# MartinPippel/DAmar

Hardware: AMD Instinct MI355X
Metric: aligned base-pairs/sec (daligner block-vs-block) (higher is better)
Workload: dtype int32

## Files before the change

damar_amd/csrc/kernels/kernels.h:

```cpp
#ifndef DAMAR_KERNELS_H
#define DAMAR_KERNELS_H

#include "dev_common.h"

size_t damar_scan_workspace_bytes(u64 n);
void   damar_exclusive_scan_u32(const u32 *in, u32 *out, u64 n, void *work, u64 *total_dev, hipStream_t st);
#define DAMAR_SCAN_TILE 4096
void   damar_tile_offsets_u32(const u32 *in, u64 n, void *work, u64 *total_dev, hipStream_t st);
void   damar_scan_tile_counts(u32 *tcount, u32 ntiles, u64 *total_dev, hipStream_t st);
size_t damar_sort_workspace_bytes(u64 n);
void   damar_sort_set_threads(int threads);
const u32 *damar_sort_error_word(const void *work);
int    damar_radix_sort_keys_u64(u64 *k0, u64 *k1, u64 n, int lobit, int hibit, void *work, hipStream_t st);
void   damar_radix_sort_split_u64(u64 *k0, u64 *k1, u64 n, int lobit, int hibit, u32 *ohi, u32 *olo, void *work,
                                  hipStream_t st);
int    damar_radix_sort_u32(u32 *k0, u32 *v0, u32 *k1, u32 *v1, u64 n, int nbits, void *work, hipStream_t st);
int    damar_radix_sort_keys_u32(u32 *k0, u32 *k1, u64 n, int nbits, void *work, hipStream_t st);
int    damar_radix_sort_u64(u64 *k0, u32 *v0, u64 *k1, u32 *v1, u64 n, int nbits, void *work, hipStream_t st);

typedef struct
{ const u8  *bases;
  const u32 *pk;
  u32        rbias;
  const u32 *boff;
// ... 64 lines not shown
  int  self, comp, identity;
  u32  limit;
  DevBlock ablk, bblk;
  int  pbits, abits;
  int  dbits;
} MergeArgs;

typedef struct { u32 b0, b1, ja, ia;
                 u32 sh, pad[3]; } MergeTile;

size_t damar_merge_workspace_bytes(u32 alen);
u32   *damar_merge_tile_counts(void *work, u32 alen);
u32    damar_merge_tiles(u32 alen);
void   damar_launch_merge_count(const MergeArgs *m, void *work, unsigned long long *gram, u32 ngram, hipStream_t st);
void damar_launch_merge_emit(const MergeArgs *m, void *work, u64 nhits, u64 *keys, u32 *vals, u32 *pid, hipStream_t st);
void damar_launch_pair_heads_ids(const u32 *pids, u64 nhits, int abits, int minhit, int nshift,
                                 u64 *send, u64 *bits, void *scan_work, u64 *total_dev, u32 *heads, hipStream_t st);
void damar_launch_pair_bitmap(const u32 *pids, const u32 *heads, u32 nheads, int abits, u32 b_lo, u32 b_hi, u32 *bitmap,
                              hipStream_t st);
void damar_launch_seed_cut_count(const u64 *keys, u64 nhits, int pbits, const u32 *bitmap, u32 *tcount, u64 *total_dev,
                                 hipStream_t st);
void damar_launch_seed_cut_scatter(const u64 *keys, const u32 *vals, u64 nhits, int pbits, const u32 *bitmap,
                                   const u32 *toff, u64 *okeys, u32 *ovals, hipStream_t st);
void damar_launch_pair_heads(const u64 *keys, u64 nhits, int pbits, int abits, int minhit, int nshift,
                             u64 *send , u64 *bits, void *scan_work, u64 *total_dev,
                             u32 *heads, hipStream_t st);
void damar_launch_pair_work(u64 *keys, const u32 *vals, u64 nhits, int ppos, int dbits, int abits, int minhit, int nshift,
                            u64 *send , u64 *bits, void *scan_work, u64 *total_dev ,
                            int binshift, int kmer, int hitmin, u32 b_lo, u32 b_hi, int unsorted, hipStream_t st);
void damar_launch_order_runs(u64 *keys, u64 nhits, int ppos, int dbits, const u32 *work, u32 nwork, hipStream_t st);
// ... 146 lines not shown
```

damar_amd/csrc/kernels/radix_sort.hip:

```cpp
#include <atomic>
#include <type_traits>
#include "dev_common.h"
#include "kernels.h"

SEED_PRIO_VAR(g_sort_prio, 1)
SEED_PRIO_SETTER(damar_sort_set_prio, g_sort_prio)

#ifndef OS_THREADS
#define OS_THREADS 1024
#endif
#ifndef OS_MINW
#define OS_MINW    4
#endif
#ifndef OS_RANK_LDS
#define OS_RANK_LDS 1
#endif
#define OS_MINTILE (256 * 8)
#define OS_MAXPASS 8

#define OH_ITEMS   16

#define LB_COUNT   1u
#define LB_PREFIX  2u
#define LB_SPINS   (1u << 24)
#ifndef LB_AHEAD
#define LB_AHEAD   8
#endif

#define WS_HIST    256
#define WS_CTR     (256 + OS_MAXPASS * 256 * 4)
#define WS_LB      16384

template <typename GT> __device__ __forceinline__ GT lb_load(const GT *p)
{ return __hip_atomic_load(p, __ATOMIC_RELAXED, __HIP_MEMORY_SCOPE_AGENT); }
template <typename GT> __device__ __forceinline__ void lb_store(GT *p, GT v)
{ __hip_atomic_store(p, v, __ATOMIC_RELAXED, __HIP_MEMORY_SCOPE_AGENT); }

__device__ __forceinline__ u32 os_scan256(u32 v, u32 *lds4)
{ const int l = lane_id(), w = threadIdx.x >> 6;
  const u32 inc = (u32) wave_incl_scan_i((int) v);
  if (l == 63 && w < 4) lds4[w] = inc;
  __syncthreads();
  u32 base = 0;
  for (int i = 0; i < 4; i++)
    if (i < w) base += lds4[i];
  __syncthreads();
  return base + inc - v;
}


#define OH_THREADS 1024
// ... 439 lines not shown
```

damar_amd/csrc/kernels/seed_merge.hip:

```cpp
#include "dev_common.h"
#include "kernels.h"

SEED_PRIO_VAR(g_merge_prio, 0)
SEED_PRIO_SETTER(damar_merge_set_prio, g_merge_prio)


__device__ __forceinline__ u32 count_below(const u32 *__restrict__ bpos, u32 jb, u32 ib, u32 bound)
{ u32 a = jb, b = ib;
  while (a < b)
    { u32 m = (a + b) >> 1;
      if (bpos[m] < bound) a = m + 1; else b = m;
    }
  return a - jb;
}


#ifndef MT_PER
#define MT_PER  4
#endif
#define MT_A    (MT_PER * 256)
#define MT_BCAP (3 * MT_A)
#define MT_HITS 4
#define MT_NBK  2048

template <typename CodeT>
__device__ __forceinline__ u32 lower_bound_c(const CodeT *c, u32 lo, u32 hi, CodeT x)
{ while (lo < hi)
    { const u32 mid = (lo + hi) >> 1;
      if (c[mid] < x) lo = mid + 1; else hi = mid;
    }
  return lo;
}
template <typename CodeT>
__device__ __forceinline__ u32 upper_bound_c(const CodeT *c, u32 lo, u32 hi, CodeT x)
{ while (lo < hi)
    { const u32 mid = (lo + hi) >> 1;
      if (c[mid] <= x) lo = mid + 1; else hi = mid;
    }
  return lo;
}

#define MT_SMP 8192
template <typename CodeT>
__global__ __launch_bounds__(256)
void merge_tiles(MergeArgs m, u32 ntiles, MergeTile *__restrict__ tiles)
{ SEED_PRIO(g_merge_prio);
  constexpr u32 NS = sizeof(CodeT) == 4 ? MT_SMP : MT_SMP / 2;
  __shared__ CodeT smp[NS];
  const CodeT *acode = (const CodeT *) m.acode, *bcode = (const CodeT *) m.bcode;
  const u32 stride = (m.blen + NS - 1) / NS;
  if (m.blen > 0)
    for (u32 j = threadIdx.x; j < NS; j += 256)
      { const u64 e = (u64) (j + 1) * stride - 1;
        smp[j] = bcode[e < m.blen ? (u32) e : m.blen - 1];
      }
  __syncthreads();
  const u32 t = blockIdx.x * 256u + threadIdx.x;
  if (t >= ntiles)
    return;
  const u32 a0 = t * (u32) MT_A, a1 = min(m.alen, a0 + (u32) MT_A);
  const CodeT c0 = acode[a0], c1 = acode[a1 - 1];
// ... 73 lines not shown
  return count_below(m.bpos, jb, jb + nb, bound);
}

__device__ __forceinline__ u64 block_sum_u64(u64 v, u64 *red)
{ for (int o = 32; o > 0; o >>= 1)
    { const u32 lo = (u32) __shfl_xor((int) (u32) v, o), hi = (u32) __shfl_xor((int) (u32) (v >> 32), o);
      v += ((u64) hi << 32) | lo;
    }
  __syncthreads();
  if (lane_id() == 0) red[threadIdx.x >> 6] = v;
  __syncthreads();
  return red[0] + red[1] + red[2] + red[3];
}

template <typename CodeT, bool INLDS>
__device__ __forceinline__ void merge_sweep_tile(const MergeArgs &m, const MergeTile tl, const u32 tile,
                                                 u32 *__restrict__ tcount, u32 *__restrict__ cnt, u32 *__restrict__ jbg,
                                                 unsigned long long *__restrict__ gram, u32 ngram,
                                                 CodeT *sb, u32 *loc, u32 *sjb, u32 *sw4, u64 *red)
{ const CodeT *acode = (const CodeT *) m.acode, *bcode = (const CodeT *) m.bcode;
  const int l = lane_id(), w = threadIdx.x >> 6;
  const u32 a0 = tile * (u32) MT_A, a1 = min(m.alen, a0 + (u32) MT_A), nat = a1 - a0;
  const u32 nbt = tl.b1 - tl.b0;
  const u32 e0 = threadIdx.x * MT_PER;
  const int nv = (e0 >= nat) ? 0 : (int) min((u32) MT_PER, nat - e0);

  constexpr u32 VPK = 16 / sizeof(CodeT);
  typedef CodeT VecT __attribute__((ext_vector_type(16 / sizeof(CodeT))));
  CodeT a[MT_PER];
  if (nv == MT_PER)
    {
// ... 242 lines not shown
#pragma unroll
      for (int k = 0; k < 4; k++)
        { vc[k] = n[k];  vj[k] = tl.b0 + jb[k]; }
      *(V4 *) (cnt + a0 + e0) = vc;
      *(V4 *) (jbg + a0 + e0) = vj;
    }
  else
    {
#pragma unroll
      for (int k = 0; k < MT_PER; k++)
        if (k < nv)
          { cnt[a0 + e0 + k] = n[k];
            jbg[a0 + e0 + k] = tl.b0 + jb[k];
          }
    }
}

static_assert(MT_BCAP + 16 < (1 << 16), "a packed entry holds the piece-relative start and the hits in 16 bits each");
struct MergeFastArgs
{ const void *acode, *bcode;
  const u32  *apos, *bpos;
  u32 alen, blen;
  int self, identity, comp, rpbits;
};

template <typename CodeT>
__global__ __launch_bounds__(256, 8)
void merge_fast(MergeFastArgs m, MergeTile *__restrict__ tiles, u32 *__restrict__ tcount, u32 *__restrict__ cnt)
{ SEED_PRIO(g_merge_prio);
  __shared__ __attribute__((aligned(16))) CodeT sb[MT_BCAP + 16 / sizeof(CodeT)];
  __shared__ __attribute__((aligned(16))) u16 first[MT_NBK];
  __shared__ u32 wsum[4];
  __shared__ u32 deep;
  const CodeT *acode = (const CodeT *) m.acode, *bcode = (const CodeT *) m.bcode;
  const u32 tile = blockIdx.x;
  const MergeTile tl = tiles[tile];
  const u32 a0 = tile * (u32) MT_A, a1 = min(m.alen, a0 + (u32) MT_A), nat = a1 - a0;
  const u32 nbt = tl.b1 - tl.b0;
  if (nbt > MT_BCAP || (m.self && m.rpbits == 0))
    { if (threadIdx.x == 0)
        tiles[tile].pad[0] = 1;
      return;
    }
  const u32 e0 = threadIdx.x * MT_PER;
  const int nv = (e0 >= nat) ? 0 : (int) min((u32) MT_PER, nat - e0);
  const u32 sh = tl.sh, nmax = tl.pad[1];
  constexpr u32 VPK = 16 / sizeof(CodeT);
  typedef CodeT VecT __attribute__((ext_vector_type(16 / sizeof(CodeT))));
  typedef u32 V4 __attribute__((ext_vector_type(4)));

  const CodeT c0 = acode[a0];
  CodeT a[MT_PER];
  if (nv == MT_PER)
    {
#pragma unroll
      for (int q = 0; q < MT_PER / (int) VPK; q++)
        { const VecT v = ((const VecT *) (acode + a0 + e0))[q];
#pragma unroll
// ... 34 lines not shown
    for (int r = 0; r < MT_BCAP / (int) VPK / 256 + 1; r++)
      { const u32 x = threadIdx.x + (u32) r * 256;
        if (x < nvec)
          ((VecT *) sb)[x] = v[r];
      }
  }
  const CodeT *B = sb + shf;
  __syncthreads();
  for (u32 j = threadIdx.x; j < nbt; j += 256)
    { const u32 bk = (u32) ((B[j] - c0) >> sh);
      if (j == 0 || (u32) ((B[j - 1] - c0) >> sh) != bk)
        first[bk] = (u16) j;
    }
  __syncthreads();

  u32 jb[MT_PER], n[MT_PER];
  u32 longest = 0;
#pragma unroll
  for (int k = 0; k < MT_PER; k++)
    { jb[k] = 0;  n[k] = 0;
      if (k < nv)
        { const CodeT c = a[k];
          if (k > 0 && c == a[k - 1])
            { jb[k] = jb[k - 1];  n[k] = n[k - 1]; }
          else
            { u32 p = first[(u32) ((c - c0) >> sh)];
              if (p != 0xffffu)
                { int steps = 0;
                  while (p < nbt && B[p] < c)
                    { p += 1;
                      if (++steps == 4) { p = lower_bound_c<CodeT>(B, p, nbt, c);  break; }
// ... 20 lines not shown
        if (n[k] > 0)
          { const u32 p = m.apos[a0 + e0 + k], ra = p >> rp;
            u32 bound = m.identity ? (m.comp ? (ra + 1) << rp : p) : ra << rp;
            if (!(m.identity && m.comp && ((ra + 1) >> (32 - rp)) != 0))
              n[k] = count_below(m.bpos, tl.b0 + jb[k], tl.b0 + jb[k] + n[k], bound);
          }
    }
#pragma unroll
  for (int k = 0; k < MT_PER; k++)
    sum += n[k];
  sum = (u32) wave_sum_i((int) sum);
  if (lane_id() == 0)
    wsum[threadIdx.x >> 6] = sum;
  __syncthreads();
  if (deep)
    { if (threadIdx.x == 0)
        tiles[tile].pad[0] = 1;
      return;
    }
  if (threadIdx.x == 0)
    { tcount[tile] = wsum[0] + wsum[1] + wsum[2] + wsum[3];
      tiles[tile].pad[2] = 1;
    }
  if (nv == MT_PER && MT_PER == 4)
    { V4 vc;
#pragma unroll
      for (int k = 0; k < 4; k++)
        vc[k] = (n[k] << 16) | jb[k];
      *(V4 *) (cnt + a0 + e0) = vc;
    }
  else
    {
#pragma unroll
      for (int k = 0; k < MT_PER; k++)
        if (k < nv)
          cnt[a0 + e0 + k] = (n[k] << 16) | jb[k];
    }
}

template <typename CodeT>
__global__ __launch_bounds__(256, 8)
void merge_sweep(MergeArgs m, const MergeTile *__restrict__ tiles, u32 *__restrict__ tcount, u32 *__restrict__ cnt,
                 u32 *__restrict__ jbg, unsigned long long *__restrict__ gram, u32 ngram, int only_flagged)
{ SEED_PRIO(g_merge_prio);
  __shared__ __attribute__((aligned(16))) CodeT sb[MT_BCAP + 16 / sizeof(CodeT)];
  __shared__ u32 loc[MT_A + 1];
  __shared__ u32 sjb[2];
  __shared__ u32 sw4[4];
  __shared__ u64 red[4];
  const MergeTile tl = tiles[blockIdx.x];
  if (only_flagged && tl.pad[0] == 0)
    return;
  if (tl.b1 - tl.b0 <= MT_BCAP)
    merge_sweep_tile<CodeT, true>(m, tl, blockIdx.x, tcount, cnt, jbg, gram, ngram, sb, loc, sjb, sw4, red);
  else
    merge_sweep_tile<CodeT, false>(m, tl, blockIdx.x, tcount, cnt, jbg, gram, ngram, sb, loc, sjb, sw4, red);
}

__global__ __launch_bounds__(256, 8)
void merge_emit(MergeArgs m, const MergeTile *__restrict__ tiles, const u32 *__restrict__ cnt, const u32 *__restrict__ jbg,
                const u32 *__restrict__ toff, u64 nhits, u64 *__restrict__ keys, u32 *__restrict__ vals, u32 *__restrict__ pid)
{ SEED_PRIO(g_merge_prio);
  __shared__ u32 loc[MT_A + 1];
  __shared__ u32 sjb[MT_A];
  __shared__ u32 sw4[4];
  const int l = lane_id(), w = threadIdx.x >> 6;
  const u32 tile = blockIdx.x;
  const u32 a0 = tile * (u32) MT_A, a1 = min(m.alen, a0 + (u32) MT_A), nat = a1 - a0;
  const u32 e0 = threadIdx.x * MT_PER;
  const u64 h0 = toff[tile];
  const u64 hn = (tile + 1 < gridDim.x) ? (u64) toff[tile + 1] : nhits;
  if (hn == h0)
    return;
  u32 n[MT_PER], s = 0;
  const bool packed = tiles[tile].pad[2] != 0;
  const u32 pb0 = tiles[tile].b0;
#pragma unroll
  for (int k = 0; k < MT_PER; k++)
    { const bool ok = e0 + k < nat;
      const u32 w = ok ? cnt[a0 + e0 + k] : 0;
      n[k] = packed ? w >> 16 : w;
      sjb[e0 + k] = !ok ? 0 : packed ? pb0 + (w & 0xffffu) : jbg[a0 + e0 + k];
      s += n[k];
    }
  u32 inc = (u32) wave_incl_scan_i((int) s);
  if (l == 63) sw4[w] = inc;
  __syncthreads();
  u32 ex = inc - s;
  for (int i = 0; i < 4; i++)
    if (i < w) ex += sw4[i];
#pragma unroll
  for (int k = 0; k < MT_PER; k++)
    { loc[e0 + k] = ex;
      ex += n[k];
    }
  if (threadIdx.x == 255)
    loc[MT_A] = ex;
  __syncthreads();
  const u32 T = loc[MT_A];
  for (u32 t0 = threadIdx.x; t0 < T; t0 += 256 * MT_HITS)
    { u32 ai[MT_HITS], bi[MT_HITS], pa[MT_HITS], pb[MT_HITS];
#pragma unroll
      for (int x = 0; x < MT_HITS; x++)
        { const u32 t = t0 + (u32) x * 256;
          u32 lo = 0, hi = MT_A;
          if (t < T)
            while (hi - lo > 1)
              { const u32 mid = (lo + hi) >> 1;
                if (loc[mid] <= t) lo = mid; else hi = mid;
              }
          ai[x] = a0 + lo;
          bi[x] = (t < T) ? sjb[lo] + (t - loc[lo]) : 0;
        }
#pragma unroll
      for (int x = 0; x < MT_HITS; x++)
        { const bool ok = t0 + (u32) x * 256 < T;
          pa[x] = ok ? m.apos[ai[x]] : 0;
          pb[x] = ok ? m.bpos[bi[x]] : 0;
        }
      u32 ra[MT_HITS], rb[MT_HITS], xa[MT_HITS], xb[MT_HITS];
      if (m.ablk.rpbits && m.bblk.rpbits)
        {
#pragma unroll
          for (int x = 0; x < MT_HITS; x++)
            { ra[x] = pa[x] >> m.ablk.rpbits;  xa[x] = pa[x] & ((1u << m.ablk.rpbits) - 1u);
              rb[x] = pb[x] >> m.bblk.rpbits;  xb[x] = pb[x] & ((1u << m.bblk.rpbits) - 1u);
            }
        }
      else
        {
#pragma unroll
          for (int x = 0; x < MT_HITS; x++)
            { pos_decode(m.ablk, pa[x], &ra[x], &xa[x]);
              pos_decode(m.bblk, pb[x], &rb[x], &xb[x]);
            }
        }
// ... 4 lines not shown
          if (t < T && h < nhits)
            { const u64 key = ((u64) rb[x] << (m.abits + m.pbits)) | ((u64) ra[x] << m.pbits) | (u64) xa[x];
              if (m.dbits)
                keys[h] = (key << m.dbits) | (u64) xb[x];
              else
                { keys[h] = key;
                  vals[h] = (u32) ((int) xa[x] - (int) xb[x]);
                }
              if (pid != NULL)
                pid[h] = (rb[x] << m.abits) | ra[x];
            }
        }
    }
}

static size_t mw_tiles(u32 alen)  { return ((size_t) alen + MT_A - 1) / MT_A; }
static size_t mw_off_counts(u32 alen) { return (mw_tiles(alen) * sizeof(MergeTile) + 255) & ~(size_t) 255; }
static size_t mw_off_cnt(u32 alen)    { return mw_off_counts(alen) + (((mw_tiles(alen) + 1) * sizeof(u32) + 255) & ~(size_t) 255); }
static size_t mw_off_jb(u32 alen)     { return mw_off_cnt(alen) + (((size_t) alen * sizeof(u32) + 255) & ~(size_t) 255); }

size_t damar_merge_workspace_bytes(u32 alen)
{ return mw_off_jb(alen) + (((size_t) alen * sizeof(u32) + 255) & ~(size_t) 255); }

u32 *damar_merge_tile_counts(void *work, u32 alen) { return (u32 *) ((char *) work + mw_off_counts(alen)); }

u32 damar_merge_tiles(u32 alen) { return (u32) mw_tiles(alen); }

void damar_launch_merge_count(const MergeArgs *m, void *work, unsigned long long *gram, u32 ngram, hipStream_t st)
{ if (m->alen == 0)
    return;
  const u32 ntiles = (u32) mw_tiles(m->alen);
  MergeTile *tiles = (MergeTile *) work;
  u32 *tcount = damar_merge_tile_counts(work, m->alen);
  u32 *cnt = (u32 *) ((char *) work + mw_off_cnt(m->alen)), *jb = (u32 *) ((char *) work + mw_off_jb(m->alen));
  static int general = -1;
  if (general < 0)
    general = getenv("DAMAR_MERGE_GENERAL") != NULL;
  const bool fast = gram == NULL && !general;
  MergeFastArgs f;
  f.acode = m->acode;  f.bcode = m->bcode;  f.apos = m->apos;  f.bpos = m->bpos;  f.alen = m->alen;  f.blen = m->blen;
  f.self = m->self;  f.identity = m->identity;  f.comp = m->comp;  f.rpbits = m->ablk.rpbits;
  if (m->wide)
    { hipLaunchKernelGGL(merge_tiles<u64>, dim3((ntiles + 255) / 256), dim3(256), 0, st, *m, ntiles, tiles);
      if (fast)
        hipLaunchKernelGGL(merge_fast<u64>, dim3(ntiles), dim3(256), 0, st, f, tiles, tcount, cnt);
      hipLaunchKernelGGL(merge_sweep<u64>, dim3(ntiles), dim3(256), 0, st, *m, tiles, tcount, cnt, jb, gram, ngram, fast ? 1 : 0);
    }
  else
    { hipLaunchKernelGGL(merge_tiles<u32>, dim3((ntiles + 255) / 256), dim3(256), 0, st, *m, ntiles, tiles);
      if (fast)
        hipLaunchKernelGGL(merge_fast<u32>, dim3(ntiles), dim3(256), 0, st, f, tiles, tcount, cnt);
      hipLaunchKernelGGL(merge_sweep<u32>, dim3(ntiles), dim3(256), 0, st, *m, tiles, tcount, cnt, jb, gram, ngram, fast ? 1 : 0);
    }
}

void damar_launch_merge_emit(const MergeArgs *m, void *work, u64 nhits, u64 *keys, u32 *vals, u32 *pid, hipStream_t st)
{ if (nhits == 0)
    return;
  const u32 ntiles = (u32) mw_tiles(m->alen);
  const u32 *toff = damar_merge_tile_counts(work, m->alen);
  const u32 *cnt = (const u32 *) ((char *) work + mw_off_cnt(m->alen)), *jb = (const u32 *) ((char *) work + mw_off_jb(m->alen));
  hipLaunchKernelGGL(merge_emit, dim3(ntiles), dim3(256), 0, st, *m, (const MergeTile *) work, cnt, jb, toff, nhits, keys, vals, pid);
}

#define SCREEN_MAX   48
#define SCREEN_PANEL 50000
template <typename K>
__global__ __launch_bounds__(64)
void slice_ends(const K *__restrict__ keys, u64 nhits, int bshift, int nshift, u64 *__restrict__ send)
{ const int nthr = 1 << nshift, t = threadIdx.x;
  if (t >= nthr)
    return;
  u64 e;
  if (t == nthr - 1)
    e = nhits;
  else
    { e = (nhits * (u64) (t + 1)) >> nshift;
      if (e > 0)
// ... 763 lines not shown
```

damar_amd/csrc/shim.hip:

```cpp
#include <algorithm>
#include <vector>
#include <deque>
#include <string>
#include <thread>
#include <atomic>
#include <mutex>
#include <condition_variable>
#include <functional>
#include <string.h>
#include <unistd.h>

#include "kernels/dev_common.h"
#include <ctype.h>
#include "kernels/kernels.h"

extern "C" {
#include "damar_filter.h"
#include "damar_hip.h"
#include "host/damar_host.h"
}

#define MAXGRAM 10000

static void die(void)
// ... 1730 lines not shown
  m.abits = std::max(1, ilog2_ceil((u64) ablock->nreads));
  int bbits = std::max(1, ilog2_ceil((u64) bblock->nreads));
  if (m.pbits + m.abits + bbits > 64)
    { fprintf(stderr, "damar: FATAL: seed key needs %d bits (> 64)\n", m.pbits + m.abits + bbits);
      die();
    }
  { static int pack_on = -1;
    if (pack_on < 0)
      { const char *e = getenv("DAMAR_PACK_SEEDS");
        pack_on = e ? atoi(e) : 1;
      }
    const int db = std::max(1, ilog2_ceil((u64) bblock->maxlen + 1));
    m.dbits = (pack_on && m.pbits + m.abits + bbits + db <= 64) ? db : 0;
  }

  const u32 mtiles = damar_merge_tiles(alen);
  void *mw;
  u32  *tcount;
  u64  *tot;
  u64   total = 0;

  if (Q_flush > 0)
    { Q_ms[3] += now_ms() - Q_flush;  Q_flush = 0; }
  Q_seg[3] += now_ms() - f->t_entry;
  tick(0);
  arena_reserve(&G_work, pad256(damar_merge_workspace_bytes(alen)) + pad256(damar_scan_workspace_bytes(mtiles)) + 4096);
  mw = arena_take(&G_work, damar_merge_workspace_bytes(alen));
  tcount = damar_merge_tile_counts(mw, alen);
  tot = (u64 *) arena_take(&G_work, 64);
  void *mscw = arena_take(&G_work, damar_scan_workspace_bytes(mtiles));
  damar_launch_merge_count(&m, mw, NULL, 0, G_st);
  stage("merge_count");
  damar_exclusive_scan_u32(tcount, tcount, mtiles, mscw, tot, G_st);
  stage("merge_scan");
  HIP_CHECK(hipMemcpyAsync(&total, tot, sizeof(u64), hipMemcpyDeviceToHost, G_st));
  stream_wait(G_st);
  if (MEM_LIMIT > 0)
    {
      int   limit = MAXGRAM;
      int64 avail = (int64) (MEM_LIMIT - (uint64) (sizeof_db(ablock) + sizeof_db(bblock))) / 16;
      if (aidx == bidx || avail > (int64) alen + 2 * (int64) blen)
        avail = (avail - alen) / 2;
      else
        avail = avail - ((int64) alen + blen);
      avail = (int64) (avail * .98);
      if ((int64) total > avail)
        { std::vector<unsigned long long> histo(MAXGRAM);
          unsigned long long *dgram = (unsigned long long *) dmalloc(sizeof(unsigned long long) * MAXGRAM);
          HIP_CHECK(hipMemsetAsync(dgram, 0, sizeof(unsigned long long) * MAXGRAM, G_st));
          damar_launch_merge_count(&m, mw, dgram, MAXGRAM, G_st);
          HIP_CHECK(hipMemcpyAsync(histo.data(), dgram, sizeof(unsigned long long) * MAXGRAM, hipMemcpyDeviceToHost, G_st));
          HIP_CHECK(hipStreamSynchronize(G_st));
          HIP_CHECK(hipFree(dgram));
          int64 tom = 0;
          int   j;
          for (j = 0; j < MAXGRAM; j++)
            { tom += (int64) j * (int64) histo[j];
              if (tom > avail)
                break;
            }
          limit = j;
          if (limit <= 1)
// ... 30 lines not shown
  else
    G_limit = 0x7fffffff;
  nhits = (int64) total;
  if (VERBOSE)
    { printf("   Hit count = %lld\n", (long long) nhits);
      fflush(stdout);
    }
  if (total >= 0xfffffff0ull)
    { fprintf(stderr, "damar: FATAL: %llu seed pairs exceed the 32-bit seed index of this build\n",
              (unsigned long long) total);
      die();
    }
  if (total == 0)
    return false;

  const int sbits = m.pbits + m.abits + bbits;
  const int spasses = (sbits + 7) / 8;
  const int minhit = (P_hitmin - 1) / P_kmer + 1;
  const int idbits = m.abits + bbits;
  static int cut_on = -1;
  if (cut_on < 0)
    { const char *e = getenv("DAMAR_EARLY_CUT");
      cut_on = e ? atoi(e) : 0;
    }
  const bool ranged = P_bread_lo > 0 || P_bread_hi != 0xffffffffu;
  const bool cut = (cut_on || ranged) && !G_keep_seeds && idbits <= 32;
  static int two_step = -1;
  if (two_step < 0)
    { const char *e = getenv("DAMAR_WORK_TWOSTEP");
      two_step = (e && atoi(e) > 0) ? 1 : 0;
    }
  static int pair_sort = -1;
  static long long pair_ratio = 4000;
  static u64 prev_seeds = 0, prev_work = 1;
  if (pair_sort < 0)
    { const char *e = getenv("DAMAR_SORT_PAIR"), *r = getenv("DAMAR_ADAPT_RATIO");
      pair_sort = e ? atoi(e) : 2;
      if (r)
        pair_ratio = atoll(r);
    }
  const bool pair_on = pair_sort == 1 || (pair_sort == 2 && pair_ratio > 0 && prev_seeds / prev_work > (u64) pair_ratio);
  bool psort = pair_on && !cut && !two_step && !G_keep_seeds && m.dbits != 0 && m.pbits + 11 <= 32 && m.pbits >= 8;
  const int spasses_used = psort ? (sbits - m.pbits + 7) / 8 : spasses;
  u64 *keys, *tk;
  u32 *vals, *flags, *foff;
  void *scw2, *resort_ws = NULL;
  u64 *sends;
  int  hshift = P_nshift;
  if (!cut)
    { arena_reserve(&G_hits, pad256(sizeof(u64) * (size_t) total) + pad256(sizeof(u32) * (size_t) total) + 4096);
      arena_reserve(&G_tmp,  pad256(sizeof(u64) * (size_t) total) + 3 * pad256(sizeof(u32) * (size_t) total) +
                             pad256(damar_sort_workspace_bytes(total)) + pad256(damar_scan_workspace_bytes(total)) + 8192);
      u64 *pk = (u64 *) arena_take(&G_hits, sizeof(u64) * (size_t) total);
      u32 *pv = m.dbits ? NULL : (u32 *) arena_take(&G_hits, sizeof(u32) * (size_t) total);
      tk = (u64 *) arena_take(&G_tmp, sizeof(u64) * (size_t) total);
      u32 *tv = m.dbits ? NULL : (u32 *) arena_take(&G_tmp, sizeof(u32) * (size_t) total);
      u64 *k0 = (spasses_used & 1) ? tk : pk, *k1 = (spasses_used & 1) ? pk : tk;
      u32 *v0 = (spasses_used & 1) ? tv : pv, *v1 = (spasses_used & 1) ? pv : tv;
      void *sw = arena_take(&G_tmp, damar_sort_workspace_bytes(total));
      resort_ws = sw;
      flags = (u32 *) arena_take(&G_tmp, sizeof(u32) * (size_t) total);
      foff  = (u32 *) arena_take(&G_tmp, std::max(sizeof(u32) * (size_t) total, bit_words_bytes(total)));
      scw2  = arena_take(&G_tmp, damar_scan_workspace_bytes(total));
      sends = (u64 *) arena_take(&G_tmp, 64 * sizeof(u64));

      damar_launch_merge_emit(&m, mw, total, k0, v0, NULL, G_st);
      stage("merge_emit");
      tick(1);
      int side = m.dbits ? damar_radix_sort_keys_u64(k0, k1, total, m.dbits + (psort ? m.pbits : 0), m.dbits + sbits, sw, G_st)
                         : damar_radix_sort_u64(k0, v0, k1, v1, total, sbits, sw, G_st);
      sort_check(sw);
      keys = side ? k1 : k0;
      vals = side ? v1 : v0;
      if (keys != pk)
        { fprintf(stderr, "damar: internal error, the seed sort ended on the wrong side\n");
          die();
        }
    }
  else
    {
      const size_t bmwords = (((size_t) 1 << idbits) + 31) / 32;
      arena_reserve(&G_tmp, pad256(sizeof(u64) * (size_t) total) + 4 * pad256(sizeof(u32) * (size_t) total) +
// ... 1507 lines not shown
```

Measured before the change: 50.67 billion.

## Add fused single-pass merge count+emit kernel with decoupled look-back

Adds a merge_fused kernel that counts seed hits per tile, computes the tile's output offset with a decoupled look-back scan, and emits keys directly. This removes the separate count, scan, host readback and emit passes. The seed buffers are sized to the arena's capacity up front, with a fallback when they overflow. The path is gated behind DAMAR_MERGE_FUSED, which defaults to off. Launch-bound occupancy for 64-bit codes also drops from 8 to 5 workgroups, which applies to the default merge_fast and merge_sweep kernels too.

```diff
diff --git a/damar_amd/csrc/kernels/kernels.h b/damar_amd/csrc/kernels/kernels.h
--- a/damar_amd/csrc/kernels/kernels.h
+++ b/damar_amd/csrc/kernels/kernels.h
@@ -102,6 +102,8 @@
 u32    damar_merge_tiles(u32 alen);
 void   damar_launch_merge_count(const MergeArgs *m, void *work, unsigned long long *gram, u32 ngram, hipStream_t st);
 void damar_launch_merge_emit(const MergeArgs *m, void *work, u64 nhits, u64 *keys, u32 *vals, u32 *pid, hipStream_t st);
+void damar_launch_merge_fused(const MergeArgs *m, void *work, u64 cap, u64 *keys, u32 *vals, u32 *pid, hipStream_t st);
+const u64 *damar_merge_fused_words(const void *work, u32 alen);
 void damar_launch_pair_heads_ids(const u32 *pids, u64 nhits, int abits, int minhit, int nshift,
                                  u64 *send, u64 *bits, void *scan_work, u64 *total_dev, u32 *heads, hipStream_t st);
 void damar_launch_pair_bitmap(const u32 *pids, const u32 *heads, u32 nheads, int abits, u32 b_lo, u32 b_hi, u32 *bitmap,
diff --git a/damar_amd/csrc/kernels/lookback.h b/damar_amd/csrc/kernels/lookback.h
--- /dev/null
+++ b/damar_amd/csrc/kernels/lookback.h
@@ -0,0 +1,50 @@
+#ifndef DAMAR_LOOKBACK_H
+#define DAMAR_LOOKBACK_H
+#include "dev_common.h"
+
+#define LB_COUNT   1u
+#define LB_PREFIX  2u
+#define LB_SPINS   (1u << 24)
+
+template <typename GT> __device__ __forceinline__ GT lb_load(const GT *p)
+{ return __hip_atomic_load(p, __ATOMIC_RELAXED, __HIP_MEMORY_SCOPE_AGENT); }
+template <typename GT> __device__ __forceinline__ void lb_store(GT *p, GT v)
+{ __hip_atomic_store(p, v, __ATOMIC_RELAXED, __HIP_MEMORY_SCOPE_AGENT); }
+
+__device__ __forceinline__ u64 lb_exclusive_u64(u64 *__restrict__ lb, u32 tile, u64 mine, u32 *__restrict__ err)
+{ constexpr int SH = 62;
+  constexpr u64 VM = (1ull << SH) - 1;
+  const int l = lane_id();
+  if (l == 0 && tile > 0)
+    lb_store<u64>(&lb[tile], ((u64) LB_COUNT << SH) | (mine & VM));
+  u64 before = 0;
+  u32 t = tile, spins = 0;
+  while (t > 0)
+    { const bool in = (u32) l < t;
+      const u64 g  = in ? lb_load<u64>(&lb[t - 1 - (u32) l]) : 0ull;
+      const u32 st = in ? (u32) (g >> SH) : LB_PREFIX;
+      const u64 pm = wballot(st == LB_PREFIX), em = wballot(st == 0);
+      const int fp = pm ? __ffsll((unsigned long long) pm) - 1 : 64, fe = em ? __ffsll((unsigned long long) em) - 1 : 64;
+      const int take = (fp < fe) ? fp + 1 : fe;
+      u64 v = (l < take) ? (g & VM) : 0ull;
+      for (int o = 32; o > 0; o >>= 1)
+        { const u32 lo = (u32) __shfl_xor((int) (u32) v, o), hi = (u32) __shfl_xor((int) (u32) (v >> 32), o);
+          v += ((u64) hi << 32) | lo;
+        }
+      before += v;
+      if (fp < fe)
+        break;
+      t -= (u32) fe;
+      if (fe < 64)
+        { if (++spins > LB_SPINS)
+            { if (l == 0) atomicOr(err, 1u);
+              break;
+            }
+          __builtin_amdgcn_s_sleep(1);
+        }
+    }
+  if (l == 0)
+    lb_store<u64>(&lb[tile], ((u64) LB_PREFIX << SH) | ((before + mine) & VM));
+  return before;
+}
+#endif
diff --git a/damar_amd/csrc/kernels/radix_sort.hip b/damar_amd/csrc/kernels/radix_sort.hip
--- a/damar_amd/csrc/kernels/radix_sort.hip
+++ b/damar_amd/csrc/kernels/radix_sort.hip
@@ -2,6 +2,7 @@
 #include <type_traits>
 #include "dev_common.h"
 #include "kernels.h"
+#include "lookback.h"
 
 SEED_PRIO_VAR(g_sort_prio, 1)
 SEED_PRIO_SETTER(damar_sort_set_prio, g_sort_prio)
@@ -20,9 +21,6 @@
 
 #define OH_ITEMS   16
 
-#define LB_COUNT   1u
-#define LB_PREFIX  2u
-#define LB_SPINS   (1u << 24)
 #ifndef LB_AHEAD
 #define LB_AHEAD   8
 #endif
@@ -30,11 +28,6 @@
 #define WS_HIST    256
 #define WS_CTR     (256 + OS_MAXPASS * 256 * 4)
 #define WS_LB      16384
-
-template <typename GT> __device__ __forceinline__ GT lb_load(const GT *p)
-{ return __hip_atomic_load(p, __ATOMIC_RELAXED, __HIP_MEMORY_SCOPE_AGENT); }
-template <typename GT> __device__ __forceinline__ void lb_store(GT *p, GT v)
-{ __hip_atomic_store(p, v, __ATOMIC_RELAXED, __HIP_MEMORY_SCOPE_AGENT); }
 
 __device__ __forceinline__ u32 os_scan256(u32 v, u32 *lds4)
 { const int l = lane_id(), w = threadIdx.x >> 6;
diff --git a/damar_amd/csrc/kernels/seed_merge.hip b/damar_amd/csrc/kernels/seed_merge.hip
--- a/damar_amd/csrc/kernels/seed_merge.hip
+++ b/damar_amd/csrc/kernels/seed_merge.hip
@@ -1,5 +1,6 @@
 #include "dev_common.h"
 #include "kernels.h"
+#include "lookback.h"
 
 SEED_PRIO_VAR(g_merge_prio, 0)
 SEED_PRIO_SETTER(damar_merge_set_prio, g_merge_prio)
@@ -22,6 +23,7 @@
 #define MT_BCAP (3 * MT_A)
 #define MT_HITS 4
 #define MT_NBK  2048
+#define MT_WGS(CodeT) (sizeof(CodeT) == 4 ? 8 : 5)
 
 template <typename CodeT>
 __device__ __forceinline__ u32 lower_bound_c(const CodeT *c, u32 lo, u32 hi, CodeT x)
@@ -41,10 +43,20 @@
 }
 
 #define MT_SMP 8192
+#define MF_WORDS  4
+#define MF_TOTAL  0
+#define MF_OVER   1
+#define MF_ERR    2
+#define MF_TICKET 3
 template <typename CodeT>
 __global__ __launch_bounds__(256)
-void merge_tiles(MergeArgs m, u32 ntiles, MergeTile *__restrict__ tiles)
+void merge_tiles(MergeArgs m, u32 ntiles, MergeTile *__restrict__ tiles, u64 *__restrict__ lb)
 { SEED_PRIO(g_merge_prio);
+  if (lb != NULL)
+    { const u32 t = blockIdx.x * 256u + threadIdx.x;
+      if (t < ntiles + MF_WORDS)
+        lb[t] = 0;
+    }
   constexpr u32 NS = sizeof(CodeT) == 4 ? MT_SMP : MT_SMP / 2;
   __shared__ CodeT smp[NS];
   const CodeT *acode = (const CodeT *) m.acode, *bcode = (const CodeT *) m.bcode;
@@ -148,7 +160,7 @@
 }
 
 template <typename CodeT, bool INLDS>
-__device__ __forceinline__ void merge_sweep_tile(const MergeArgs &m, const MergeTile tl, const u32 tile,
+__device__ __forceinline__ u64 merge_sweep_tile(const MergeArgs &m, const MergeTile tl, const u32 tile,
                                                  u32 *__restrict__ tcount, u32 *__restrict__ cnt, u32 *__restrict__ jbg,
                                                  unsigned long long *__restrict__ gram, u32 ngram,
                                                  CodeT *sb, u32 *loc, u32 *sjb, u32 *sw4, u64 *red)
@@ -421,6 +433,7 @@
             jbg[a0 + e0 + k] = tl.b0 + jb[k];
           }
     }
+  return T64;
 }
 
 static_assert(MT_BCAP + 16 < (1 << 16), "a packed entry holds the piece-relative start and the hits in 16 bits each");
@@ -432,23 +445,15 @@
 };
 
 template <typename CodeT>
-__global__ __launch_bounds__(256, 8)
-void merge_fast(MergeFastArgs m, MergeTile *__restrict__ tiles, u32 *__restrict__ tcount, u32 *__restrict__ cnt)
-{ SEED_PRIO(g_merge_prio);
-  __shared__ __attribute__((aligned(16))) CodeT sb[MT_BCAP + 16 / sizeof(CodeT)];
-  __shared__ __attribute__((aligned(16))) u16 first[MT_NBK];
-  __shared__ u32 wsum[4];
-  __shared__ u32 deep;
+__device__ __forceinline__ bool merge_fast_tile(const MergeFastArgs &m, const MergeTile &tl, const u32 tile,
+                                                CodeT *sb, u16 *first, u32 *wsum, u32 *deepp,
+                                                u32 (&jb)[MT_PER], u32 (&n)[MT_PER], u32 *T)
+{ u32 &deep = *deepp;
   const CodeT *acode = (const CodeT *) m.acode, *bcode = (const CodeT *) m.bcode;
-  const u32 tile = blockIdx.x;
-  const MergeTile tl = tiles[tile];
   const u32 a0 = tile * (u32) MT_A, a1 = min(m.alen, a0 + (u32) MT_A), nat = a1 - a0;
   const u32 nbt = tl.b1 - tl.b0;
   if (nbt > MT_BCAP || (m.self && m.rpbits == 0))
-    { if (threadIdx.x == 0)
-        tiles[tile].pad[0] = 1;
-      return;
-    }
+    return false;
   const u32 e0 = threadIdx.x * MT_PER;
   const int nv = (e0 >= nat) ? 0 : (int) min((u32) MT_PER, nat - e0);
   const u32 sh = tl.sh, nmax = tl.pad[1];
@@ -513,7 +518,6 @@
     }
   __syncthreads();
 
-  u32 jb[MT_PER], n[MT_PER];
   u32 longest = 0;
 #pragma unroll
   for (int k = 0; k < MT_PER; k++)
@@ -564,12 +568,33 @@
     wsum[threadIdx.x >> 6] = sum;
   __syncthreads();
   if (deep)
+    return false;
+  *T = wsum[0] + wsum[1] + wsum[2] + wsum[3];
+  return true;
+}
+
+template <typename CodeT>
+__global__ __launch_bounds__(256, MT_WGS(CodeT))
+void merge_fast(MergeFastArgs m, MergeTile *__restrict__ tiles, u32 *__restrict__ tcount, u32 *__restrict__ cnt)
+{ SEED_PRIO(g_merge_prio);
+  __shared__ __attribute__((aligned(16))) CodeT sb[MT_BCAP + 16 / sizeof(CodeT)];
+  __shared__ __attribute__((aligned(16))) u16 first[MT_NBK];
+  __shared__ u32 wsum[4];
+  __shared__ u32 deep;
+  typedef u32 V4 __attribute__((ext_vector_type(4)));
+  const u32 tile = blockIdx.x;
+  const MergeTile tl = tiles[tile];
+  const u32 a0 = tile * (u32) MT_A, a1 = min(m.alen, a0 + (u32) MT_A), nat = a1 - a0;
+  const u32 e0 = threadIdx.x * MT_PER;
+  const int nv = (e0 >= nat) ? 0 : (int) min((u32) MT_PER, nat - e0);
+  u32 jb[MT_PER], n[MT_PER], T;
+  if (!merge_fast_tile<CodeT>(m, tl, tile, sb, first, wsum, &deep, jb, n, &T))
     { if (threadIdx.x == 0)
         tiles[tile].pad[0] = 1;
       return;
     }
   if (threadIdx.x == 0)
-    { tcount[tile] = wsum[0] + wsum[1] + wsum[2] + wsum[3];
+    { tcount[tile] = T;
       tiles[tile].pad[2] = 1;
     }
   if (nv == MT_PER && MT_PER == 4)
@@ -589,7 +614,7 @@
 }
 
 template <typename CodeT>
-__global__ __launch_bounds__(256, 8)
+__global__ __launch_bounds__(256, MT_WGS(CodeT))
 void merge_sweep(MergeArgs m, const MergeTile *__restrict__ tiles, u32 *__restrict__ tcount, u32 *__restrict__ cnt,
                  u32 *__restrict__ jbg, unsigned long long *__restrict__ gram, u32 ngram, int only_flagged)
 { SEED_PRIO(g_merge_prio);
@@ -607,24 +632,12 @@
     merge_sweep_tile<CodeT, false>(m, tl, blockIdx.x, tcount, cnt, jbg, gram, ngram, sb, loc, sjb, sw4, red);
 }
 
-__global__ __launch_bounds__(256, 8)
-void merge_emit(MergeArgs m, const MergeTile *__restrict__ tiles, const u32 *__restrict__ cnt, const u32 *__restrict__ jbg,
-                const u32 *__restrict__ toff, u64 nhits, u64 *__restrict__ keys, u32 *__restrict__ vals, u32 *__restrict__ pid)
-{ SEED_PRIO(g_merge_prio);
-  __shared__ u32 loc[MT_A + 1];
-  __shared__ u32 sjb[MT_A];
-  __shared__ u32 sw4[4];
-  const int l = lane_id(), w = threadIdx.x >> 6;
-  const u32 tile = blockIdx.x;
-  const u32 a0 = tile * (u32) MT_A, a1 = min(m.alen, a0 + (u32) MT_A), nat = a1 - a0;
+
+__device__ __forceinline__ void emit_stage_tile(const u32 *__restrict__ cnt, const u32 *__restrict__ jbg, const bool packed,
+                                                const u32 pb0, const u32 a0, const u32 nat, u32 *loc, u32 *sjb, u32 *sw4)
+{ const int l = lane_id(), w = threadIdx.x >> 6;
   const u32 e0 = threadIdx.x * MT_PER;
-  const u64 h0 = toff[tile];
-  const u64 hn = (tile + 1 < gridDim.x) ? (u64) toff[tile + 1] : nhits;
-  if (hn == h0)
-    return;
   u32 n[MT_PER], s = 0;
-  const bool packed = tiles[tile].pad[2] != 0;
-  const u32 pb0 = tiles[tile].b0;
 #pragma unroll
   for (int k = 0; k < MT_PER; k++)
     { const bool ok = e0 + k < nat;
@@ -647,8 +660,13 @@
   if (threadIdx.x == 255)
     loc[MT_A] = ex;
   __syncthreads();
-  const u32 T = loc[MT_A];
-  for (u32 t0 = threadIdx.x; t0 < T; t0 += 256 * MT_HITS)
+}
+
+template <bool RP>
+__device__ __forceinline__ void emit_tile(const MergeArgs &m, const u32 a0, const u32 T, const u64 h0, const u64 nhits,
+                                          const u32 *loc, const u32 *sjb,
+                                          u64 *__restrict__ keys, u32 *__restrict__ vals, u32 *__restrict__ pid)
+{ for (u32 t0 = threadIdx.x; t0 < T; t0 += 256 * MT_HITS)
     { u32 ai[MT_HITS], bi[MT_HITS], pa[MT_HITS], pb[MT_HITS];
 #pragma unroll
       for (int x = 0; x < MT_HITS; x++)
@@ -669,7 +687,7 @@
           pb[x] = ok ? m.bpos[bi[x]] : 0;
         }
       u32 ra[MT_HITS], rb[MT_HITS], xa[MT_HITS], xb[MT_HITS];
-      if (m.ablk.rpbits && m.bblk.rpbits)
+      if (RP || (m.ablk.rpbits && m.bblk.rpbits))
         {
 #pragma unroll
           for (int x = 0; x < MT_HITS; x++)
@@ -704,13 +722,118 @@
     }
 }
 
+__global__ __launch_bounds__(256, 8)
+void merge_emit(MergeArgs m, const MergeTile *__restrict__ tiles, const u32 *__restrict__ cnt, const u32 *__restrict__ jbg,
+                const u32 *__restrict__ toff, u64 nhits, u64 *__restrict__ keys, u32 *__restrict__ vals, u32 *__restrict__ pid)
+{ SEED_PRIO(g_merge_prio);
+  __shared__ u32 loc[MT_A + 1];
+  __shared__ u32 sjb[MT_A];
+  __shared__ u32 sw4[4];
+  const u32 tile = blockIdx.x;
+  const u32 a0 = tile * (u32) MT_A, a1 = min(m.alen, a0 + (u32) MT_A), nat = a1 - a0;
+  const u64 h0 = toff[tile];
+  const u64 hn = (tile + 1 < gridDim.x) ? (u64) toff[tile + 1] : nhits;
+  if (hn == h0)
+    return;
+  emit_stage_tile(cnt, jbg, tiles[tile].pad[2] != 0, tiles[tile].b0, a0, nat, loc, sjb, sw4);
+  emit_tile<false>(m, a0, loc[MT_A], h0, nhits, loc, sjb, keys, vals, pid);
+}
+
+template <typename CodeT>
+__global__ __launch_bounds__(256, MT_WGS(CodeT))
+void merge_fused(MergeArgs m, const MergeTile *__restrict__ tiles, u32 ntiles, u32 *__restrict__ tcount, u32 *__restrict__ cnt,
+                 u32 *__restrict__ jbg, u64 *__restrict__ lb, u64 cap, int general,
+                 u64 *__restrict__ keys, u32 *__restrict__ vals, u32 *__restrict__ pid)
+{ SEED_PRIO(g_merge_prio);
+  __shared__ __attribute__((aligned(16))) CodeT sb[MT_BCAP + 16 / sizeof(CodeT)];
+  __shared__ __attribute__((aligned(16))) u32 loc[MT_A + 4];
+  __shared__ u32 sjb2[2];
+  __shared__ u32 sw4[4];
+  __shared__ u64 red[4];
+  __shared__ u32 deep;
+  __shared__ u32 s_tile;
+  __shared__ u64 s_before;
+  static_assert(sizeof(u16) * MT_NBK <= sizeof(u32) * MT_A, "the table does not fit the prefix");
+  static_assert(sizeof(CodeT) * MT_BCAP >= sizeof(u32) * MT_A, "the B-run starts do not fit the stage");
+  u32 *const sjb = (u32 *) sb;
+  u64 *const ctl = lb + ntiles;
+  if (threadIdx.x == 0)
+    s_tile = atomicAdd((u32 *) &ctl[MF_TICKET], 1u);
+  __syncthreads();
+  const u32 tile = (u32) __builtin_amdgcn_readfirstlane((int) s_tile);
+  const MergeTile tl = tiles[tile];
+  const u32 a0 = tile * (u32) MT_A, a1 = min(m.alen, a0 + (u32) MT_A), nat = a1 - a0;
+  const u32 e0 = threadIdx.x * MT_PER;
+
+  u64 T = 0;
+  bool fast = !general && m.ablk.rpbits != 0 && m.bblk.rpbits != 0;
+  if (fast)
+    { MergeFastArgs f;
+      f.acode = m.acode;  f.bcode = m.bcode;  f.apos = m.apos;  f.bpos = m.bpos;  f.alen = m.alen;  f.blen = m.blen;
+      f.self = m.self;  f.identity = m.identity;  f.comp = m.comp;  f.rpbits = m.ablk.rpbits;
+      u32 jb[MT_PER], n[MT_PER], T32 = 0;
+      fast = merge_fast_tile<CodeT>(f, tl, tile, sb, (u16 *) loc, sw4, &deep, jb, n, &T32);
+      if (fast)
+        { u32 s = 0;
+#pragma unroll
+          for (int k = 0; k < MT_PER; k++)
+            s += n[k];
+          u32 ex = (u32) wave_incl_scan_i((int) s) - s;
+          for (int i = 0; i < 4; i++)
+            if (i < (int) (threadIdx.x >> 6)) ex += sw4[i];
+#pragma unroll
+          for (int k = 0; k < MT_PER; k++)
+            { loc[e0 + k] = ex;
+              sjb[e0 + k] = tl.b0 + jb[k];
+              ex += n[k];
+            }
+          if (threadIdx.x == 255)
+            loc[MT_A] = ex;
+          T = T32;
+        }
+    }
+  if (!fast)
+    { __syncthreads();
+      if (tl.b1 - tl.b0 <= MT_BCAP)
+        T = merge_sweep_tile<CodeT, true>(m, tl, tile, tcount, cnt, jbg, NULL, 0, sb, loc, sjb2, sw4, red);
+      else
+        T = merge_sweep_tile<CodeT, false>(m, tl, tile, tcount, cnt, jbg, NULL, 0, sb, loc, sjb2, sw4, red);
+    }
+
+  if (threadIdx.x < 64)
+    { const u64 before = lb_exclusive_u64(lb, tile, T, (u32 *) &ctl[MF_ERR]);
+      if (threadIdx.x == 0)
+        { s_before = before;
+          if (tile == ntiles - 1)
+            ctl[MF_TOTAL] = before + T;
+        }
+    }
+  __syncthreads();
+  const u64 h0 = s_before;
+  if (T == 0)
+    return;
+  if (h0 + T > cap || T > 0xffffffffull)
+    { if (threadIdx.x == 0)
+        ctl[MF_OVER] = 1;
+      return;
+    }
+  if (fast)
+    emit_tile<true>(m, a0, (u32) T, h0, cap, loc, sjb, keys, vals, pid);
+  else
+    { emit_stage_tile(cnt, jbg, false, 0, a0, nat, loc, sjb, sw4);
+      emit_tile<false>(m, a0, (u32) T, h0, cap, loc, sjb, keys, vals, pid);
+    }
+}
+
 static size_t mw_tiles(u32 alen)  { return ((size_t) alen + MT_A - 1) / MT_A; }
 static size_t mw_off_counts(u32 alen) { return (mw_tiles(alen) * sizeof(MergeTile) + 255) & ~(size_t) 255; }
 static size_t mw_off_cnt(u32 alen)    { return mw_off_counts(alen) + (((mw_tiles(alen) + 1) * sizeof(u32) + 255) & ~(size_t) 255); }
 static size_t mw_off_jb(u32 alen)     { return mw_off_cnt(alen) + (((size_t) alen * sizeof(u32) + 255) & ~(size_t) 255); }
 
+static size_t mw_off_lb(u32 alen)     { return mw_off_jb(alen) + (((size_t) alen * sizeof(u32) + 255) & ~(size_t) 255); }
+
 size_t damar_merge_workspace_bytes(u32 alen)
-{ return mw_off_jb(alen) + (((size_t) alen * sizeof(u32) + 255) & ~(size_t) 255); }
+{ return mw_off_lb(alen) + (((mw_tiles(alen) + MF_WORDS) * sizeof(u64) + 255) & ~(size_t) 255); }
 
 u32 *damar_merge_tile_counts(void *work, u32 alen) { return (u32 *) ((char *) work + mw_off_counts(alen)); }
 
@@ -731,13 +854,13 @@
   f.acode = m->acode;  f.bcode = m->bcode;  f.apos = m->apos;  f.bpos = m->bpos;  f.alen = m->alen;  f.blen = m->blen;
   f.self = m->self;  f.identity = m->identity;  f.comp = m->comp;  f.rpbits = m->ablk.rpbits;
   if (m->wide)
-    { hipLaunchKernelGGL(merge_tiles<u64>, dim3((ntiles + 255) / 256), dim3(256), 0, st, *m, ntiles, tiles);
+    { hipLaunchKernelGGL(merge_tiles<u64>, dim3((ntiles + 255) / 256), dim3(256), 0, st, *m, ntiles, tiles, (u64 *) NULL);
       if (fast)
         hipLaunchKernelGGL(merge_fast<u64>, dim3(ntiles), dim3(256), 0, st, f, tiles, tcount, cnt);
       hipLaunchKernelGGL(merge_sweep<u64>, dim3(ntiles), dim3(256), 0, st, *m, tiles, tcount, cnt, jb, gram, ngram, fast ? 1 : 0);
     }
   else
-    { hipLaunchKernelGGL(merge_tiles<u32>, dim3((ntiles + 255) / 256), dim3(256), 0, st, *m, ntiles, tiles);
+    { hipLaunchKernelGGL(merge_tiles<u32>, dim3((ntiles + 255) / 256), dim3(256), 0, st, *m, ntiles, tiles, (u64 *) NULL);
       if (fast)
         hipLaunchKernelGGL(merge_fast<u32>, dim3(ntiles), dim3(256), 0, st, f, tiles, tcount, cnt);
       hipLaunchKernelGGL(merge_sweep<u32>, dim3(ntiles), dim3(256), 0, st, *m, tiles, tcount, cnt, jb, gram, ngram, fast ? 1 : 0);
@@ -752,6 +875,33 @@
   const u32 *cnt = (const u32 *) ((char *) work + mw_off_cnt(m->alen)), *jb = (const u32 *) ((char *) work + mw_off_jb(m->alen));
   hipLaunchKernelGGL(merge_emit, dim3(ntiles), dim3(256), 0, st, *m, (const MergeTile *) work, cnt, jb, toff, nhits, keys, vals, pid);
 }
+
+void damar_launch_merge_fused(const MergeArgs *m, void *work, u64 cap, u64 *keys, u32 *vals, u32 *pid, hipStream_t st)
+{ if (m->alen == 0)
+    return;
+  const u32 ntiles = (u32) mw_tiles(m->alen);
+  MergeTile *tiles = (MergeTile *) work;
+  u32 *tcount = damar_merge_tile_counts(work, m->alen);
+  u32 *cnt = (u32 *) ((char *) work + mw_off_cnt(m->alen)), *jb = (u32 *) ((char *) work + mw_off_jb(m->alen));
+  u64 *lb = (u64 *) ((char *) work + mw_off_lb(m->alen));
+  static int general = -1;
+  if (general < 0)
+    general = getenv("DAMAR_MERGE_GENERAL") != NULL;
+  const u32 nclear = ntiles + MF_WORDS;
+  if (m->wide)
+    { hipLaunchKernelGGL(merge_tiles<u64>, dim3((nclear + 255) / 256), dim3(256), 0, st, *m, ntiles, tiles, lb);
+      hipLaunchKernelGGL(merge_fused<u64>, dim3(ntiles), dim3(256), 0, st, *m, tiles, ntiles, tcount, cnt, jb, lb, cap, general,
+                         keys, vals, pid);
+    }
+  else
+    { hipLaunchKernelGGL(merge_tiles<u32>, dim3((nclear + 255) / 256), dim3(256), 0, st, *m, ntiles, tiles, lb);
+      hipLaunchKernelGGL(merge_fused<u32>, dim3(ntiles), dim3(256), 0, st, *m, tiles, ntiles, tcount, cnt, jb, lb, cap, general,
+                         keys, vals, pid);
+    }
+}
+
+const u64 *damar_merge_fused_words(const void *work, u32 alen)
+{ return (const u64 *) ((const char *) work + mw_off_lb(alen)) + mw_tiles(alen); }
 
 #define SCREEN_MAX   48
 #define SCREEN_PANEL 50000
diff --git a/damar_amd/csrc/shim.hip b/damar_amd/csrc/shim.hip
--- a/damar_amd/csrc/shim.hip
+++ b/damar_amd/csrc/shim.hip
@@ -1768,6 +1768,71 @@
     m.dbits = (pack_on && m.pbits + m.abits + bbits + db <= 64) ? db : 0;
   }
 
+  const int sbits = m.pbits + m.abits + bbits;
+  const int spasses = (sbits + 7) / 8;
+  const int minhit = (P_hitmin - 1) / P_kmer + 1;
+  const int idbits = m.abits + bbits;
+  static int cut_on = -1;
+  if (cut_on < 0)
+    { const char *e = getenv("DAMAR_EARLY_CUT");
+      cut_on = e ? atoi(e) : 0;
+    }
+  const bool ranged = P_bread_lo > 0 || P_bread_hi != 0xffffffffu;
+  const bool cut = (cut_on || ranged) && !G_keep_seeds && idbits <= 32;
+  static int two_step = -1;
+  if (two_step < 0)
+    { const char *e = getenv("DAMAR_WORK_TWOSTEP");
+      two_step = (e && atoi(e) > 0) ? 1 : 0;
+    }
+  static int pair_sort = -1;
+  static long long pair_ratio = 4000;
+  static u64 prev_seeds = 0, prev_work = 1;
+  if (pair_sort < 0)
+    { const char *e = getenv("DAMAR_SORT_PAIR"), *r = getenv("DAMAR_ADAPT_RATIO");
+      pair_sort = e ? atoi(e) : 2;
+      if (r)
+        pair_ratio = atoll(r);
+    }
+  const bool pair_on = pair_sort == 1 || (pair_sort == 2 && pair_ratio > 0 && prev_seeds / prev_work > (u64) pair_ratio);
+  bool psort = pair_on && !cut && !two_step && !G_keep_seeds && m.dbits != 0 && m.pbits + 11 <= 32 && m.pbits >= 8;
+  const int spasses_used = psort ? (sbits - m.pbits + 7) / 8 : spasses;
+
+  static int fused_on = -1;
+  static long long test_cap = -1;
+  if (fused_on < 0)
+    { const char *e = getenv("DAMAR_MERGE_FUSED"), *c = getenv("DAMAR_TEST_MERGE_CAP");
+      fused_on = e ? (atoi(e) != 0) : 0;
+      if (c)
+        test_cap = atoll(c);
+    }
+  const bool fused = fused_on && !cut;
+  bool emitted = false;
+  u64  lay = 0;
+  u64 *keys, *tk, *k0 = NULL, *k1 = NULL;
+  u32 *vals, *v0 = NULL, *v1 = NULL;
+  auto hits_need = [&](u64 n) { return pad256(sizeof(u64) * (size_t) n) + pad256(sizeof(u32) * (size_t) n) + 4096; };
+  auto tmp_need  = [&](u64 n) { return pad256(sizeof(u64) * (size_t) n) + 3 * pad256(sizeof(u32) * (size_t) n) +
+                                       pad256(damar_sort_workspace_bytes(n)) + pad256(damar_scan_workspace_bytes(n)) + 8192; };
+  auto lay_seeds = [&](u64 n)
+    { lay = n;
+      arena_reserve(&G_hits, hits_need(n));
+      arena_reserve(&G_tmp,  tmp_need(n));
+      u64 *pk = (u64 *) arena_take(&G_hits, sizeof(u64) * (size_t) n);
+      u32 *pv = m.dbits ? NULL : (u32 *) arena_take(&G_hits, sizeof(u32) * (size_t) n);
+      tk = (u64 *) arena_take(&G_tmp, sizeof(u64) * (size_t) n);
+      u32 *tv = m.dbits ? NULL : (u32 *) arena_take(&G_tmp, sizeof(u32) * (size_t) n);
+      k0 = (spasses_used & 1) ? tk : pk;  k1 = (spasses_used & 1) ? pk : tk;
+      v0 = (spasses_used & 1) ? tv : pv;  v1 = (spasses_used & 1) ? pv : tv;
+    };
+  auto room = [&]() -> u64
+    { u64 lo = 0, hi = 0xffffffefull;
+      while (lo < hi)
+        { const u64 mid = lo + (hi - lo + 1) / 2;
+          if (hits_need(mid) <= G_hits.cap && tmp_need(mid) <= G_tmp.cap) lo = mid; else hi = mid - 1;
+        }
+      return lo;
+    };
+
   const u32 mtiles = damar_merge_tiles(alen);
   void *mw;
   u32  *tcount;
@@ -1783,12 +1848,35 @@
   tcount = damar_merge_tile_counts(mw, alen);
   tot = (u64 *) arena_take(&G_work, 64);
   void *mscw = arena_take(&G_work, damar_scan_workspace_bytes(mtiles));
-  damar_launch_merge_count(&m, mw, NULL, 0, G_st);
-  stage("merge_count");
-  damar_exclusive_scan_u32(tcount, tcount, mtiles, mscw, tot, G_st);
-  stage("merge_scan");
-  HIP_CHECK(hipMemcpyAsync(&total, tot, sizeof(u64), hipMemcpyDeviceToHost, G_st));
-  stream_wait(G_st);
+  auto sweep_fused = [&](u64 n) -> bool
+    { u64 res[3] = { 0, 0, 0 };
+      lay_seeds(n);
+      damar_launch_merge_fused(&m, mw, n, k0, v0, NULL, G_st);
+      stage("merge_fused");
+      HIP_CHECK(hipMemcpyAsync(res, damar_merge_fused_words(mw, alen), sizeof(res), hipMemcpyDeviceToHost, G_st));
+      stream_wait(G_st);
+      if (res[2] != 0)
+        { fprintf(stderr, "damar: FATAL: the merge's look-back timed out\n");
+          die();
+        }
+      total = res[0];
+      return res[1] == 0;
+    };
+  if (fused)
+    { u64 n = room();
+      if (test_cap >= 0 && (u64) test_cap < n)
+        n = (u64) test_cap;
+      emitted = sweep_fused(n);
+    }
+  else
+    { damar_launch_merge_count(&m, mw, NULL, 0, G_st);
+      stage("merge_count");
+      damar_exclusive_scan_u32(tcount, tcount, mtiles, mscw, tot, G_st);
+      stage("merge_scan");
+      HIP_CHECK(hipMemcpyAsync(&total, tot, sizeof(u64), hipMemcpyDeviceToHost, G_st));
+      stream_wait(G_st);
+    }
+  bool two_sweeps = !fused;
   if (MEM_LIMIT > 0)
     {
       int   limit = MAXGRAM;
@@ -1799,7 +1887,9 @@
         avail = avail - ((int64) alen + blen);
       avail = (int64) (avail * .98);
       if ((int64) total > avail)
-        { std::vector<unsigned long long> histo(MAXGRAM);
+        { two_sweeps = true;
+          emitted = false;
+          std::vector<unsigned long long> histo(MAXGRAM);
           unsigned long long *dgram = (unsigned long long *) dmalloc(sizeof(unsigned long long) * MAXGRAM);
           HIP_CHECK(hipMemsetAsync(dgram, 0, sizeof(unsigned long long) * MAXGRAM, G_st));
           damar_launch_merge_count(&m, mw, dgram, MAXGRAM, G_st);
@@ -1860,49 +1950,22 @@
   if (total == 0)
     return false;
 
-  const int sbits = m.pbits + m.abits + bbits;
-  const int spasses = (sbits + 7) / 8;
-  const int minhit = (P_hitmin - 1) / P_kmer + 1;
-  const int idbits = m.abits + bbits;
-  static int cut_on = -1;
-  if (cut_on < 0)
-    { const char *e = getenv("DAMAR_EARLY_CUT");
-      cut_on = e ? atoi(e) : 0;
-    }
-  const bool ranged = P_bread_lo > 0 || P_bread_hi != 0xffffffffu;
-  const bool cut = (cut_on || ranged) && !G_keep_seeds && idbits <= 32;
-  static int two_step = -1;
-  if (two_step < 0)
-    { const char *e = getenv("DAMAR_WORK_TWOSTEP");
-      two_step = (e && atoi(e) > 0) ? 1 : 0;
-    }
-  static int pair_sort = -1;
-  static long long pair_ratio = 4000;
-  static u64 prev_seeds = 0, prev_work = 1;
-  if (pair_sort < 0)
-    { const char *e = getenv("DAMAR_SORT_PAIR"), *r = getenv("DAMAR_ADAPT_RATIO");
-      pair_sort = e ? atoi(e) : 2;
-      if (r)
-        pair_ratio = atoll(r);
-    }
-  const bool pair_on = pair_sort == 1 || (pair_sort == 2 && pair_ratio > 0 && prev_seeds / prev_work > (u64) pair_ratio);
-  bool psort = pair_on && !cut && !two_step && !G_keep_seeds && m.dbits != 0 && m.pbits + 11 <= 32 && m.pbits >= 8;
-  const int spasses_used = psort ? (sbits - m.pbits + 7) / 8 : spasses;
-  u64 *keys, *tk;
-  u32 *vals, *flags, *foff;
+  u32 *flags, *foff;
   void *scw2, *resort_ws = NULL;
   u64 *sends;
   int  hshift = P_nshift;
   if (!cut)
-    { arena_reserve(&G_hits, pad256(sizeof(u64) * (size_t) total) + pad256(sizeof(u32) * (size_t) total) + 4096);
-      arena_reserve(&G_tmp,  pad256(sizeof(u64) * (size_t) total) + 3 * pad256(sizeof(u32) * (size_t) total) +
-                             pad256(damar_sort_workspace_bytes(total)) + pad256(damar_scan_workspace_bytes(total)) + 8192);
-      u64 *pk = (u64 *) arena_take(&G_hits, sizeof(u64) * (size_t) total);
-      u32 *pv = m.dbits ? NULL : (u32 *) arena_take(&G_hits, sizeof(u32) * (size_t) total);
-      tk = (u64 *) arena_take(&G_tmp, sizeof(u64) * (size_t) total);
-      u32 *tv = m.dbits ? NULL : (u32 *) arena_take(&G_tmp, sizeof(u32) * (size_t) total);
-      u64 *k0 = (spasses_used & 1) ? tk : pk, *k1 = (spasses_used & 1) ? pk : tk;
-      u32 *v0 = (spasses_used & 1) ? tv : pv, *v1 = (spasses_used & 1) ? pv : tv;
+    { if (!emitted && !two_sweeps)
+        { const u64 before = total;
+          if (!sweep_fused(total) || total != before)
+            { fprintf(stderr, "damar: internal error, the merge did not fit arenas sized for it\n");
+              die();
+            }
+          emitted = true;
+        }
+      else if (!emitted)
+        lay_seeds(total);
+      u64 *const pk = (spasses_used & 1) ? k1 : k0;
       void *sw = arena_take(&G_tmp, damar_sort_workspace_bytes(total));
       resort_ws = sw;
       flags = (u32 *) arena_take(&G_tmp, sizeof(u32) * (size_t) total);
@@ -1910,8 +1973,10 @@
       scw2  = arena_take(&G_tmp, damar_scan_workspace_bytes(total));
       sends = (u64 *) arena_take(&G_tmp, 64 * sizeof(u64));
 
-      damar_launch_merge_emit(&m, mw, total, k0, v0, NULL, G_st);
-      stage("merge_emit");
+      if (!emitted)
+        { damar_launch_merge_emit(&m, mw, total, k0, v0, NULL, G_st);
+          stage("merge_emit");
+        }
       tick(1);
       int side = m.dbits ? damar_radix_sort_keys_u64(k0, k1, total, m.dbits + (psort ? m.pbits : 0), m.dbits + sbits, sw, G_st)
                          : damar_radix_sort_u64(k0, v0, k1, v1, total, sbits, sw, G_st);
```

New measurement: 50.39 billion (median of 2 runs). No clear change (-0.6%).
